# JinPLu/VeloxSeg

Hardware: AMD Instinct MI355X
Metric: training patches/s on 128^3 2-mod volumes (fwd+loss+bwd+allreduce+AdamW) (higher is better)
Workload: dtype f32

## Files before the change

include/veloxseg_hip.h:

```cpp
#ifndef VELOXSEG_HIP_H
#define VELOXSEG_HIP_H

#ifdef __cplusplus
extern "C" {
#endif

#define VX_ABI_VERSION 1

int vx_abi_version(void);
const char* vx_last_error(void);

int vx_conv3d_fwd(const float* x, const float* x2, int C1, const float* w, const float* bias, float* y,
                  int B, int Cin, int Di, int Hi, int Wi, int Cout, int K, int S, int P, int G, int ps, void* stream);
int vx_conv3d_bwd_data(const float* dy, const float* w, const float* bias_like, float* dx, float* dx2, int C1,
                       int B, int Cin, int Di, int Hi, int Wi, int Cout, int K, int S, int P, int G, int ps,
                       int accumulate, void* stream);
int vx_conv3d_bwd_weight(const float* x, const float* x2, int C1, const float* dy, float* dw, float* db,
                         int B, int Cin, int Di, int Hi, int Wi, int Cout, int K, int S, int P, int G, int ps, void* stream);

int vx_conv3d_bwd_weight_tiled(const float* x, const float* x2, int C1, const float* dy, float* dw, float* db,
                               int B, int Cin, int Di, int Hi, int Wi, int Cout, int K, int S, int P, int G, int ps, void* stream);
int vx_down_wgrad_ws_floats(int B, int Cin, int Di, int Hi, int Wi, int Cout);
int vx_down_wgrad_mfma(const float* x, const float* dy, float* dw, float* db, float* ws, long ws_floats,
                       int B, int Cin, int Di, int Hi, int Wi, int Cout, void* stream);
// ... 223 lines not shown
                       const void* seed_ptr, unsigned long long dstream, float p_drop, void* mbits, void* stream);
int vx_pwa_attn_bwd_mb(const float* q, const float* k, const float* v, const float* table, const float* out, const float* lse, const float* dout,
                       float* dq, float* dk, float* dv, float* dtable, float* delta_ws, const VxPwaPlan* plan, int B, int M, int cq, int cv,
                       const void* seed_ptr, unsigned long long dstream, float p_drop, const void* mbits, void* stream);
int vx_pwa_attn_bwd_nofold_mb(const float* q, const float* k, const float* v, const float* table, const float* out, const float* lse, const float* dout,
                              float* dq, float* dk, float* dv, float* delta_ws, const VxPwaPlan* plan, int B, int M, int cq, int cv,
                              const void* seed_ptr, unsigned long long dstream, float p_drop, const void* mbits, void* stream);
int vx_pwa_attn_mfma_ok(const VxPwaPlan* plan, int B, int M, int cq, int cv);
int vx_pwa_attn_set_mfma(int on);
int vx_pwa_attn_bwd1h_ok(const VxPwaPlan* plan, int B, int M, int cq, int cv);
int vx_pwa_attn_set_f16_bwd(int on);
int vx_pwa_attn_set_f16_bwd_ragged(int on);
int vx_pwa_attn_set_f16_bwd_m1(int on);
int vx_pwa_attn_set_short(int on);

int vx_seg_loss_fwd(const float* l0, const float* l1, const float* l2, const float* l3, int nh, const void* labels, int lab_kind,
                    double* acc, int B, int C, long V, void* stream);
int vx_sqdiff_sum(const float* a, const float* b, long n, double* acc, void* stream);
int vx_sqdiff_sum_bs(const float* a, const float* b, long n_per_sample, long b_batch_stride, int B, double* acc, void* stream);
int vx_mse_bwd_bs(const float* a, const float* b, long n_per_sample, long b_batch_stride, int B, const float* coef, const float* gout, float* da, void* stream);
int vx_sqdiff_sum_grad_bs(const float* a, const float* b, long n_per_sample, long b_batch_stride, int B, double* acc, float scale, float* da, void* stream);
int vx_sqdiff_sum_grad_bs_h(const void* a, const float* b, long n_per_sample, long b_batch_stride, int B, double* acc, float scale, void* da, int a_h16, void* stream);
int vx_loss_finalize(const double* seg_acc, int nh, int B, int C, long V, const float* head_weights,
                     const double* rc_acc, long n_rc, float w_rc,
                     const float* gram_seg, const float* g0, const float* g1, const float* g2, const float* g3, int M, int Cg, float w_f,
                     float* loss_out, float* coef, void* stream);
int vx_seg_loss_bwd(const float* logits, const void* labels, int lab_kind, const float* coef_head, const float* gout,
                    float* dlogits, int B, int C, long V, void* stream);
int vx_seg_loss_bwd4(const float* lg0, const float* lg1, const float* lg2, const float* lg3, int nh, const void* labels, int lab_kind, const float* coef,
                     int coef_stride, const float* gout, float* dl0, float* dl1, float* dl2, float* dl3, int B, int C, long V, void* stream);
int vx_seg_loss_ds_ok(int C, int D, int H, int W);
int vx_seg_loss_ds_set_columns(int on);
int vx_seg_loss_ds_ws_floats(const int* low_dims, int nh, int B, int C, int D);
int vx_seg_loss_ds_fwd(const float* l0, const float* l1, const float* l2, const float* l3, const int* low_dims, int nh, const void* labels, int lab_kind,
                       double* acc, int B, int C, int D, int H, int W, void* stream);
int vx_seg_loss_ds_bwd(const float* l0, const float* l1, const float* l2, const float* l3, const int* low_dims, int nh, const void* labels, int lab_kind,
                       const float* coef, int coef_stride, const float* gout, float* dl0, float* dl1, float* dl2, float* dl3, float* ws,
                       int B, int C, int D, int H, int W, void* stream);
int vx_seg_loss_ds_h16_ok(const int* low_dims, int nh, int B, int C, int D, int H, int W);
int vx_seg_loss_ds_fwd_h(const void* l0, const float* l1, const float* l2, const float* l3, const int* low_dims, int nh, const void* labels, int lab_kind,
                         double* acc, int B, int C, int D, int H, int W, int l0_h16, void* stream);
int vx_seg_loss_ds_bwd_h(const void* l0, const float* l1, const float* l2, const float* l3, const int* low_dims, int nh, const void* labels, int lab_kind,
                         const float* coef, int coef_stride, const float* gout, void* dl0, float* dl1, float* dl2, float* dl3, float* ws,
                         int B, int C, int D, int H, int W, int l0_h16, void* stream);
int vx_mse_bwd(const float* a, const float* b, const float* coef, const float* gout, float* da, long n, void* stream);
int vx_gram_mse_bwd(const float* gs, const float* g0, const float* g1, const float* g2, const float* g3, int M, const float* coef,
                    const float* gout, float* dgs, float* d0, float* d1, float* d2, float* d3, long n, void* stream);
int vx_gram_fwd(const float* x, float* G, int B, int C, long V, void* stream);
int vx_gram_bwd(const float* x, const float* dG, float* dx, int B, int C, long V, void* stream);
int vx_upsample_trilinear_fwd(const float* x, float* out, long BC, int d, int h, int w, int D, int H, int W, void* stream);
int vx_upsample_trilinear_bwd(const float* dout, float* dx, float* ws, long BC, int d, int h, int w, int D, int H, int W, void* stream);

int vx_upconv_set_mfma4(int on);
int vx_upconv_k2s2_fwd(const float* x, const float* w, const float* bias, float* y, int B, int Ci, int Co, int d, int h, int wd, void* stream);
int vx_upconv_k2s2_bwd_data(const float* dy, const float* w, float* dx, int B, int Ci, int Co, int d, int h, int wd, void* stream);
int vx_upconv_k2s2_wgrad_ok(int Ci, int Co);
int vx_upconv_k2s2_wgrad(const float* x, const float* dy, float* dw, int B, int Ci, int Co, int d, int h, int wd, void* stream);

int vx_adamw_step(float* p, const float* g, float* m, float* v, long n, float lr, float beta1, float beta2, float eps,
                  float weight_decay, long step, float grad_scale, void* stream);
int vx_grad_sqnorm_blocks(void);
int vx_grad_sqnorm_partials(const float* g, long n, double* ws, void* stream);
int vx_adamw_step_ex(float* p, const float* g, float* m, float* v, long n, float lr, float beta1, float beta2, float eps, float weight_decay, long step,
                     float grad_scale, const double* ws, int nws, float max_norm, float* stats, int write_stats, float* ema, float one_minus_decay,
                     const unsigned char* chunk_group, const float* group_lr, const float* group_wd, int ngroups, void* stream);

int vx_sw_extract(const float* vol, float* win, int C, int D, int H, int W, int rd, int rh, int rw, int z0, int y0, int x0, void* stream);
int vx_sw_accumulate(const float* win, float* acc, int C, int D, int H, int W, int rd, int rh, int rw, int z0, int y0, int x0, float weight, void* stream);
int vx_sw_finalize(const float* acc, float* out, unsigned char* labels, const float* cz, const float* cy, const float* cx,
                   int C, int D, int H, int W, void* stream);
#define VX_SW_MAX_WINDOWS 16
int vx_sw_extract_mirror(const float* vol, float* win, const int* table, int nwin, int mask, int B, int C, int D, int H, int W, int rd, int rh, int rw, void* stream);
int vx_sw_mirror_sum(const float* pred, float* wsum, long rows, int rd, int rh, int rw, int mask, int first, void* stream);
int vx_sw_mirror_accumulate(const float* pred, const float* wsum, float* acc, int C, int D, int H, int W, int rd, int rh, int rw, int z0, int y0, int x0,
                            int mask, float weight, void* stream);
int vx_sw_blend_accumulate(const float* pred, const float* wsum, float* acc, const float* g, float floor, int C, int D, int H, int W, int rd, int rh, int rw,
                           int z0, int y0, int x0, int mask, float weight, void* stream);
int vx_sw_blend_finalize(const float* acc, float* out, unsigned char* labels, const float* gc, float floor, const int* tab, int cz, int cy, int cx,
                         int C, int D, int H, int W, void* stream);
int vx_argmax_channels(const float* logits, unsigned char* labels, int B, int C, long V, void* stream);
int vx_confusion(const void* pred, int pred_bytes, const void* gt, int gt_bytes, unsigned long long* conf, int B, long V, int NC, void* stream);

int vx_min_value(const float* x, long n, float* out_init_inf, void* stream);
int vx_bbox_gt(const float* x, float thr, int C, int D, int H, int W, int* out6, void* stream);
int vx_label_chunk_count(const void* labels, int lab_bytes, long n, int chunk, int fg, int* counts, void* stream);
int vx_label_kth_in_chunk(const void* labels, int lab_bytes, long n, long chunk_start, int chunk, int fg, int k, long* out_index, void* stream);
int vx_rotate_z(const float* x, float* out, int C, int D, int H, int W, float cos_a, float sin_a, int mode, void* stream);

#define VX_AUG_RECORD_BYTES 192
#define VX_AUG_MAX_STEPS 8
#define VX_AUG_LABEL (-1)
#define VX_AUG_NOISE_STREAM 0x564158475541ull
int vx_augment_batch(const void* records, int n_image, int n_label, float* x_out, void* y_out, int label_bytes, int B, int M, int D, int H, int W, void* stream);

int vx_moments_blocks(void);
int vx_moments_ws_doubles(void);
int vx_moments_partials(const float* x, long n, const float* thr, const void* mask, int mask_bytes, const double* center, double* ws, void* stream);
int vx_moments_reduce(const double* ws, double* acc, int accumulate, double* stats, int phase, void* stream);
int vx_moments_stats(const float* x, long n, const float* thr, double* ws, double* stats, void* stream);
int vx_normalize_apply(const float* x, float* out, long n, const float* thr, const double* stats, float mean, float std, int clip, float lo, float hi,
                       int policy, float floor, void* stream);
int vx_key_histogram(const float* x, const void* mask, int mask_bytes, long n, long prefix, int prefix_bits, int bin_bits, unsigned long long* hist,
                     unsigned int* minmax_key, unsigned long long* nan_count, void* stream);
int vx_resample_axes(const float* x, float* out, int C, int D, int H, int W, int Do, int Ho, int Wo, const int* i0, const int* i1, const float* w, int mode, void* stream);
int vx_resample_axes_label(const void* x, void* out, int lab_bytes, int C, int D, int H, int W, int Do, int Ho, int Wo, const int* i0, void* stream);
int vx_native_argmax(const float* logits, unsigned char* labels, int C, int D, int H, int W, int Do, int Ho, int Wo, const int* i0, const int* i1, const float* w, void* stream);

int vx_cc_ws_bytes(int D, int H, int W);
int vx_cc_grid_cap(void);
int vx_cc_label(const void* labels, int lab_bytes, int* cc, int D, int H, int W, int connectivity, void* ws, int* num, void* stream);
int vx_cc_tally(const int* cc, const void* other, int other_bytes, long V, int N, unsigned long long* sizes, unsigned long long* hits, void* stream);
int vx_cc_select(const int* cc, const unsigned char* keep, int N, const void* in, void* out, int lab_bytes, long V, void* stream);

int vx_conv_mfma_ok(int Cin, int Cout, int D, int H, int W, int K, int S, int P, int G, int ps);
int vx_conv_mfma_set_stem_f16(int on);
int vx_conv_mfma_set_stem_pieces(int np);
int vx_conv_mfma_stem_pieces(void);
int vx_conv_mfma_ws_floats(int Cin, int Cout, int K, int backward);
int vx_conv_mfma_fwd(const float* x, const float* w, const float* bias, float* y, float* ws, int B, int Cin, int D, int H, int W, int Cout, int K, int S, int P,
                     void* stream);
int vx_conv_mfma_fwd_writes_absmax(int Cin, int Cout, int D, int H, int W, int K, int S, int P);
int vx_conv_mfma_fwd_mx(const float* x, const float* w, const float* bias, float* y, float* ws, unsigned* x_absmax, int B, int Cin, int D, int H, int W, int Cout,
                        int K, int S, int P, void* stream);
int vx_conv_mfma_bwd_data(const float* dy, const float* w, float* dx, float* ws, int B, int Cin, int D, int H, int W, int Cout, int K, int S, int P, int accumulate,
                          void* stream);

int vx_expand_split_ws_floats(int Cc, int ns);
int vx_expand_fwd_mfma_split(const float* x, const float* w, const float* bias, float* wt_ws, float* y, int B, int Cc, int D, int H, int W, int ns, void* stream);
int vx_expand_bwd_data_mfma_split(const float* dy_fine, const float* w, float* wt_ws, float* dx, int B, int Cc, int D, int H, int W, int accumulate, int ns, void* stream);
int vx_expand_split_ew_offset(int Cc);
int vx_expand_prep_split22(const float* w, float* wt_fwd, float* wt_bwd, int Cc, void* stream);
int vx_expand_fwd_mfma_split_prepared(const float* x, const float* bias, const float* wt_fwd, float* y, int B, int Cc, int D, int H, int W, void* stream);
int vx_expand_bwd_data_mfma_split_prepared(const float* dy_fine, const float* wt_bwd, const float* ew_fwd, float* dx, int B, int Cc, int D, int H, int W, int accumulate, void* stream);
int vx_expand_bwd_data_mfma_split_ew(const float* dy_fine, const float* w, float* wt_ws, float* dx, int B, int Cc, int D, int H, int W, int accumulate, int ns,
                                     const float* ew_fwd, void* stream);

int vx_ln_pw_ok(int C, int NS, const int* J, long V, int s2d);
int vx_ln_pw_tiles(int B, long V);
int vx_ln_pw_fwd(const void* const* ptrs, int M, int NS, const int* J, int B, int C, long V, float eps, int s2d, int gd, int gh, int gw, void* stream);
int vx_ln_pw_bwd(const void* const* ptrs, int M, int NS, const int* J, int B, int C, long V, float eps, int s2d, int gd, int gh, int gw, void* stream);
int vx_pwa_post_ok(int C, int Cv, int R, long V);
int vx_pwa_post_tiles(int B, long V);
int vx_pwa_post_fwd(const void* const* ptrs, int M, int B, int C, int Cv, int R, long V, float eps, float alpha, const void* seed_ptr, float p_mix, float p_ffn, void* stream);
int vx_pwa_post_bwd(const void* const* ptrs, int M, int B, int C, int Cv, int R, long V, float eps, float alpha, const void* seed_ptr, float p_mix, float p_ffn, void* stream);

int vx_inmlp_ok(int C, int R, long V);
int vx_inmlp_tiles(long V);
int vx_inmlp_fwd(const float* o, const double* part, int nparts, float* stats, const float* w1, const float* b1, const float* w2, const float* b2, float* out,
                 int B, int C, int R, long V, float eps, const void* seed_ptr, unsigned long long site, float p_drop, void* stream);
int vx_inmlp_bwd(const float* o, const float* stats, const float* w1, const float* b1, const float* w2, const float* dout, float* dn, float* part_dn,
                 float* sc_n, float* sc_h, float* sc_da, float* sc_dz, int B, int C, int R, long V, const void* seed_ptr, unsigned long long site, float p_drop,
                 void* stream);
int vx_pw_wgrad_group(const void* const* ptrs, const long* dims, int nj, const void* const* fptrs, const int* fdims, int nf, void* stream);

typedef struct VxTape VxTape;
int vx_tape_build(void* hip_graph, int max_lanes, VxTape** out);
int vx_tape_build_pgo(void* graph, int max_lanes, const float* dur_us, int n, VxTape** out);
int vx_tape_info(const VxTape* tape, int* n_nodes, int* n_kernels, int* n_lanes, int* n_events);
int vx_tape_set_lane_rotation(VxTape* tape, int k);
int vx_tape_replay(VxTape* tape, void* stream);
int vx_tape_free(VxTape* tape);
int vx_tape_flag_set(void* flag, int value, void* stream);
int vx_tape_flag_wait(const void* flag, int value, void* stream);
int vx_tape_set_flags(int on);
int vx_tape_set_flag_timeout_ms(int ms);
int vx_tape_flag_timeouts(void);
int vx_tape_hop(int slot, void* src, void* dst);
int vx_tape_mark(int id, void* stream);
int vx_tape_wait_marker(VxTape* tape, int id, void* stream);
int vx_tape_has_marker(const VxTape* tape, int id);
int vx_tape_profile(VxTape* tape, void* stream, int reps, float* us);
int vx_tape_describe(const VxTape* tape, int* lane, int* grid, int* waits4, char* names, int name_stride);
int vx_tape_waits(const VxTape* tape, int* waits, int stride);
int vx_tape_launch_node(VxTape* tape, int node, void* stream);
int vx_tape_set_fuzz(int seed, float max_us, float prob);
int vx_tape_node_param(const VxTape* tape, int node, int k, int nparams, int size, void* out, int cap, int* got);
int vx_tape_node_kind(const VxTape* tape, int node);
int vx_tape_replay_prefix(VxTape* tape, void* stream, int k);
int vx_tape_lane_stream(void* any_stream, int lane, void** out);
int vx_spin_us(float us, void* stream);
int vx_tape_lanes_distinct(void);
int vx_tape_spin_us(void);
int vx_tape_lane_on_caller_queue(void);
int vx_tape_permute_lanes(const int* perm4);

#ifdef __cplusplus
}
#endif
#endif
```

veloxseg_amd/csrc/pointwise.hip:

```cpp
#include "vx_common.h"
#include "../../include/veloxseg_hip.h"
#include <type_traits>

typedef float vx_f32x4 __attribute__((ext_vector_type(4)));

template <typename TX>
__device__ __forceinline__ const TX* vx_pw_row(const TX* __restrict__ x, const TX* __restrict__ x2, int C1, int Cin, int b, int c, long V) {
    return (c < C1) ? x + ((long)b * C1 + c) * V : x2 + ((long)b * (Cin - C1) + (c - C1)) * V;
}

struct VxPwEpi {
    int mode;
    float* aux;
    VxDrop drop;
    float alpha;
};
__device__ __forceinline__ float vx_pw_epi(const VxPwEpi& e, float val, long idx) {
    if (e.mode == 1) { e.aux[idx] = val; return vx_gelu(val) * vx_drop(e.drop, (uint64_t)idx); }
    if (e.mode == 2) return val * vx_drop(e.drop, (uint64_t)idx) * vx_gelu_grad(e.aux[idx]);
    if (e.mode == 3) return fmaf(e.alpha, e.aux[idx], val * vx_drop(e.drop, (uint64_t)idx));
    return val;
}
static inline VxPwEpi vx_no_epi() { VxPwEpi e; e.mode = 0; e.aux = nullptr; e.drop.seed_ptr = nullptr; e.drop.stream = 0; e.drop.p = 0.0f; e.alpha = 1.0f; return e; }

// ... 663 lines not shown
        float4 bv[4];
#pragma unroll
        for (int s = 0; s < 4; ++s) {
            const int k = k0 + 4 * s + q;
            const bool k_ok = k < kend;
            av[s] = (m_ok && k_ok) ? wrow[(long)k * wsk] : 0.0f;
            const float* srow = (k < S1) ? src + ((long)b * S1 + k) * V : src2 + ((long)b * (Kch - S1) + (k - S1)) * V;
            bv[s] = (v_ok && k_ok) ? *reinterpret_cast<const float4*>(srow + v_b) : make_float4(0.f, 0.f, 0.f, 0.f);
        }
#pragma unroll
        for (int s = 0; s < 4; ++s) {
            acc[0] = __builtin_amdgcn_mfma_f32_16x16x4f32(av[s], bv[s].x, acc[0], 0, 0, 0);
            acc[1] = __builtin_amdgcn_mfma_f32_16x16x4f32(av[s], bv[s].y, acc[1], 0, 0, 0);
            acc[2] = __builtin_amdgcn_mfma_f32_16x16x4f32(av[s], bv[s].z, acc[2], 0, 0, 0);
            acc[3] = __builtin_amdgcn_mfma_f32_16x16x4f32(av[s], bv[s].w, acc[3], 0, 0, 0);
        }
    }
    if (ksplit > 1) {
#pragma unroll
        for (int j = 0; j < 4; ++j)
#pragma unroll
            for (int reg = 0; reg < 4; ++reg) vx_ksum4[wave][(j * 4 + reg) * 64 + lane] = acc[j][reg];
        __syncthreads();
        if (wave != 0 || !live) return;
#pragma unroll
        for (int j = 0; j < 4; ++j)
#pragma unroll
            for (int reg = 0; reg < 4; ++reg) {
                const int e = (j * 4 + reg) * 64 + lane;
                acc[j][reg] = (vx_ksum4[0][e] + vx_ksum4[1][e]) + (vx_ksum4[2][e] + vx_ksum4[3][e]);
            }
    }
    if (!v_ok) return;
#pragma unroll
    for (int reg = 0; reg < 4; ++reg) {
        const int m = mt * 16 + 4 * q + reg;
        if (m < Mch) {
            float* drow = (m < D1) ? dst + ((long)b * D1 + m) * V : dst2 + ((long)b * (Mch - D1) + (m - D1)) * V;
            const float bb = bias ? bias[m] : 0.0f;
            float4 o = make_float4(acc[0][reg] + bb, acc[1][reg] + bb, acc[2][reg] + bb, acc[3][reg] + bb);
            if (epi.mode) {
                const long idx = ((long)b * Mch + m) * V + v_b;
                if (epi.mode == 1) *reinterpret_cast<float4*>(epi.aux + idx) = o;
                const float4 ax = epi.mode >= 2 ? *reinterpret_cast<const float4*>(epi.aux + idx) : o;
                if (epi.mode == 3) {
                    o.x = fmaf(epi.alpha, ax.x, o.x * vx_drop(epi.drop, (uint64_t)idx));
                    o.y = fmaf(epi.alpha, ax.y, o.y * vx_drop(epi.drop, (uint64_t)idx + 1));
                    o.z = fmaf(epi.alpha, ax.z, o.z * vx_drop(epi.drop, (uint64_t)idx + 2));
                    o.w = fmaf(epi.alpha, ax.w, o.w * vx_drop(epi.drop, (uint64_t)idx + 3));
                } else if (epi.mode == 1) {
                    o.x = vx_gelu(ax.x) * vx_drop(epi.drop, (uint64_t)idx);
                    o.y = vx_gelu(ax.y) * vx_drop(epi.drop, (uint64_t)idx + 1);
                    o.z = vx_gelu(ax.z) * vx_drop(epi.drop, (uint64_t)idx + 2);
                    o.w = vx_gelu(ax.w) * vx_drop(epi.drop, (uint64_t)idx + 3);
                } else {
                    o.x = o.x * vx_drop(epi.drop, (uint64_t)idx) * vx_gelu_grad(ax.x);
                    o.y = o.y * vx_drop(epi.drop, (uint64_t)idx + 1) * vx_gelu_grad(ax.y);
                    o.z = o.z * vx_drop(epi.drop, (uint64_t)idx + 2) * vx_gelu_grad(ax.z);
                    o.w = o.w * vx_drop(epi.drop, (uint64_t)idx + 3) * vx_gelu_grad(ax.w);
                }
            }
            float4* dp = reinterpret_cast<float4*>(drow + v_b);
            if (accumulate) { const float4 old = *dp; o.x += old.x; o.y += old.y; o.z += old.z; o.w += old.w; }
            *dp = o;
        }
    }
}
__global__ void __launch_bounds__(256) vx_pw_mfma4_k(const float* __restrict__ src, const float* __restrict__ src2, int S1,
                                                     const float* __restrict__ w, int wsm, int wsk, const float* __restrict__ bias,
                                                     float* __restrict__ dst, float* __restrict__ dst2, int D1,
                                                     int Mch, int Kch, long V, int B, int n_vt, int accumulate, int ksplit, VxPwEpi epi) {
    vx_pw_mfma4_body(blockIdx.x, blockIdx.y, src, src2, S1, w, wsm, wsk, bias, dst, dst2, D1, Mch, Kch, V, B, n_vt, accumulate, ksplit, epi);
}

static int vx_pw_mfma4_enabled = 1;
extern "C" int vx_pw_mfma_set_wide(int on) { vx_pw_mfma4_enabled = on ? 1 : 0; return 0; }

static inline int vx_pw_ksplit(long wave_tiles, int Kch) { return (wave_tiles < 2048 && Kch >= 64) ? 4 : 1; }

static int vx_pw_conv_mfma_impl(const float* src, const float* src2, int S1, const float* w, int transpose_w, const float* bias,
                                float* dst, float* dst2, int D1, int B, int Mch, int Kch, int Cin_of_w, long V, int accumulate, void* stream, const VxPwEpi& epi) {
    VX_REQUIRE(src && w && dst && B > 0 && Mch > 0 && Kch > 0 && V > 0, "vx_pw_conv_mfma: bad args");
    if (S1 <= 0 || S1 > Kch) S1 = Kch;
    if (D1 <= 0 || D1 > Mch) D1 = Mch;
    VX_REQUIRE((S1 == Kch || src2) && (D1 == Mch || dst2), "vx_pw_conv_mfma: second tensor of a concat is missing");
    const int wsm = transpose_w ? 1 : Cin_of_w, wsk = transpose_w ? Cin_of_w : 1;
    if ((V & 3) == 0 && vx_pw_mfma4_enabled) {
        const int n_vt4 = vx_cdiv(V, 64);
        const int ks4 = vx_pw_ksplit((long)B * n_vt4 * vx_cdiv(Mch, 16), Kch);
        dim3 g4(ks4 > 1 ? (unsigned)((long)B * n_vt4) : vx_cdiv((long)B * n_vt4, 4), vx_cdiv(Mch, 16));
        vx_pw_mfma4_k<<<g4, 256, 0, (hipStream_t)stream>>>(src, src2, S1, w, wsm, wsk, bias, dst, dst2, D1, Mch, Kch, V, B, n_vt4, accumulate, ks4, epi);
        VX_LAUNCH_CHECK("vx_pw_conv_mfma");
        return 0;
    }
    const int n_vt = vx_cdiv(V, 16);
    const int ksplit = vx_pw_ksplit((long)B * n_vt * vx_cdiv(Mch, 16), Kch);
    dim3 grid(ksplit > 1 ? (unsigned)((long)B * n_vt) : vx_cdiv((long)B * n_vt, 4), vx_cdiv(Mch, 16));
    vx_pw_mfma_k<<<grid, 256, 0, (hipStream_t)stream>>>(src, src2, S1, w, wsm, wsk, bias, dst, dst2, D1, Mch, Kch, V, B, n_vt, accumulate, 0, 0, 0, 0, ksplit, epi);
    VX_LAUNCH_CHECK("vx_pw_conv_mfma");
    return 0;
}

extern "C" int vx_pw_conv_mfma(const float* src, const float* src2, int S1, const float* w, int transpose_w, const float* bias,
                               float* dst, float* dst2, int D1, int B, int Mch, int Kch, int Cin_of_w, long V, int accumulate, void* stream) {
    return vx_pw_conv_mfma_impl(src, src2, S1, w, transpose_w, bias, dst, dst2, D1, B, Mch, Kch, Cin_of_w, V, accumulate, stream, vx_no_epi());
}

__global__ void __launch_bounds__(256) vx_pw_bwd_fused_k(const float* __restrict__ dy, const float* __restrict__ w, float* __restrict__ dx, float* __restrict__ dx2,
                                                         int C1, int Cin, int Cout, long V, int B, int n_vt, int accumulate, int ksplit, int n1, int gx1,
                                                         const float* __restrict__ x, const float* __restrict__ x2, float* __restrict__ dw, float* __restrict__ db,
                                                         int vox_per_wave, int chunks_per_b, int n_ci_tiles, int gx2) {
    const int id = blockIdx.x;
    if (id < n1) {
        VxPwEpi e; e.mode = 0; e.aux = nullptr; e.drop.seed_ptr = nullptr; e.drop.stream = 0; e.drop.p = 0.0f; e.alpha = 1.0f;
        vx_pw_mfma4_body(id % gx1, id / gx1, dy, nullptr, Cout, w, 1, Cin, nullptr, dx, dx2, C1, Cin, Cout, V, B, n_vt, accumulate, ksplit, e);
    } else {
        const int j = id - n1;
        vx_pw_wgrad_body(j % gx2, j / gx2, x, x2, C1, Cin, dy, Cout, V, B, dw, db, vox_per_wave, chunks_per_b, n_ci_tiles);
    }
}

extern "C" int vx_pw_conv_bwd_fused(const float* dy, const float* w, const float* x, const float* x2, int C1, float* dx, float* dx2, float* dw, float* db,
                                    int B, int Cin, int Cout, long V, int accumulate, void* stream) {
    VX_REQUIRE(dy && w && x && dx && dw && B > 0 && Cin > 0 && Cout > 0 && V > 0, "vx_pw_conv_bwd_fused: bad args");
    if (C1 <= 0 || C1 > Cin) C1 = Cin;
    VX_REQUIRE(C1 == Cin || (x2 && dx2), "vx_pw_conv_bwd_fused: second tensor of a concat is missing");
    if ((V & 3) != 0 || !vx_pw_mfma4_enabled) {
        if (int e = vx_pw_conv_mfma_impl(dy, nullptr, 0, w, 1, nullptr, dx, dx2, C1, B, Cin, Cout, Cin, V, accumulate, stream, vx_no_epi())) return e;
        return vx_pw_conv_bwd_weight(x, x2, C1, dy, dw, db, B, Cin, Cout, V, stream);
    }
    const int n_vt4 = vx_cdiv(V, 64);
    const int ks4 = vx_pw_ksplit((long)B * n_vt4 * vx_cdiv(Cin, 16), Cout);
    const int gx1 = ks4 > 1 ? (int)((long)B * n_vt4) : vx_cdiv((long)B * n_vt4, 4), gy1 = vx_cdiv(Cin, 16);
    const int mt = vx_cdiv(Cout, 16), nt = vx_cdiv(Cin, 16);
    long waves_per_tile = 1024 / ((long)mt * nt);
    if (waves_per_tile < 4) waves_per_tile = 4;
    long vpw = ((long)B * V + waves_per_tile - 1) / waves_per_tile;
    vpw = (vpw + 63) / 64 * 64;
    if (vpw < 256) vpw = 256;
    const int chunks_per_b = vx_cdiv(V, vpw);
    const int gx2 = vx_cdiv((long)B * chunks_per_b, 4), gy2 = mt * nt;
    const long n1 = (long)gx1 * gy1, n2 = (long)gx2 * gy2;
    VX_REQUIRE(n1 + n2 < 0x7fffffffL, "vx_pw_conv_bwd_fused: grid too large");
    vx_pw_bwd_fused_k<<<dim3((unsigned)(n1 + n2)), 256, 0, (hipStream_t)stream>>>(dy, w, dx, dx2, C1, Cin, Cout, V, B, n_vt4, accumulate, ks4, (int)n1, gx1,
                                                                               x, x2, dw, db, (int)vpw, chunks_per_b, nt, gx2);
    VX_LAUNCH_CHECK("vx_pw_conv_bwd_fused");
    return 0;
}

struct VxWgJob { const float* x; const float* dy; float* dw; float* db; int Cin, Cout; long V; int B, vpw, chunks_per_b, nt, gx, blk0, nblk; };
struct VxFoldJob { const float* part; float* dg; float* dbeta; int C, rows, blk0, nblk; };
#define VX_WGG_JOBS 24
#define VX_WGG_FOLDS 16
struct VxWgGroup { VxWgJob j[VX_WGG_JOBS]; VxFoldJob f[VX_WGG_FOLDS]; int nj, nf; };
__global__ void __launch_bounds__(256) vx_pw_wgrad_group_k(VxWgGroup g) {
    const int id = blockIdx.x;
    for (int k = 0; k < g.nj; ++k) {
        const VxWgJob& J = g.j[k];
        if (id >= J.blk0 && id < J.blk0 + J.nblk) {
            const int l = id - J.blk0;
            vx_pw_wgrad_body<float>(l % J.gx, l / J.gx, J.x, (const float*)nullptr, J.Cin, J.Cin, J.dy, J.Cout, J.V, J.B, J.dw, J.db, J.vpw, J.chunks_per_b, J.nt);
            return;
        }
    }
    for (int k = 0; k < g.nf; ++k) {
        const VxFoldJob& F = g.f[k];
        if (id >= F.blk0 && id < F.blk0 + F.nblk) {
            const int r0 = (id - F.blk0) * 64, r1 = min(F.rows, r0 + 64), n = 2 * F.C;
            const int P = n < 256 ? n : 256, G = 256 / P;
            const int ci = threadIdx.x % P, gi = threadIdx.x / P;
            if (gi >= G) return;
            for (int i = ci; i < n; i += P) {
                float acc = 0.0f;
                int rr = r0 + gi;
                for (; rr + 7 * G < r1; rr += 8 * G) {
                    float t[8];
#pragma unroll
                    for (int u = 0; u < 8; ++u) t[u] = F.part[(long)(rr + u * G) * n + i];
                    acc += ((t[0] + t[1]) + (t[2] + t[3])) + ((t[4] + t[5]) + (t[6] + t[7]));
                }
                for (; rr < r1; rr += G) acc += F.part[(long)rr * n + i];
                atomicAdd(i < F.C ? F.dg + i : F.dbeta + (i - F.C), acc);
            }
            return;
        }
    }
}

extern "C" int vx_pw_wgrad_group(const void* const* ptrs, const long* dims, int nj, const void* const* fptrs, const int* fdims, int nf, void* stream) {
    VX_REQUIRE(nj >= 0 && nj <= VX_WGG_JOBS && nf >= 0 && nf <= VX_WGG_FOLDS && (nj + nf) > 0 && (nj == 0 || (ptrs && dims)) && (nf == 0 || (fptrs && fdims)), "vx_pw_wgrad_group: bad args");
    VxWgGroup g = {};
    g.nj = nj; g.nf = nf;
    long blk = 0;
    for (int k = 0; k < nj; ++k) {
        VxWgJob& J = g.j[k];
        J.x = (const float*)ptrs[4 * k]; J.dy = (const float*)ptrs[4 * k + 1]; J.dw = (float*)ptrs[4 * k + 2]; J.db = (float*)ptrs[4 * k + 3];
        J.Cin = (int)dims[4 * k]; J.Cout = (int)dims[4 * k + 1]; J.V = dims[4 * k + 2]; J.B = (int)dims[4 * k + 3];
        VX_REQUIRE(J.x && J.dy && J.dw && J.Cin > 0 && J.Cout > 0 && J.V > 0 && J.B > 0, "vx_pw_wgrad_group: bad job %d", k);
        const int mt = vx_cdiv(J.Cout, 16), nt = vx_cdiv(J.Cin, 16);
        constexpr int wgg_waves = 1024, wgg_minv = 256;
        long waves_per_tile = wgg_waves / ((long)mt * nt);
        if (waves_per_tile < 4) waves_per_tile = 4;
        long vpw = ((long)J.B * J.V + waves_per_tile - 1) / waves_per_tile;
        vpw = (vpw + 63) / 64 * 64;
        if (vpw < wgg_minv) vpw = wgg_minv;
        J.vpw = (int)vpw; J.chunks_per_b = vx_cdiv(J.V, vpw); J.nt = nt;
        J.gx = vx_cdiv((long)J.B * J.chunks_per_b, 4);
        J.blk0 = (int)blk; J.nblk = J.gx * mt * nt;
        blk += J.nblk;
    }
    for (int k = 0; k < nf; ++k) {
        VxFoldJob& F = g.f[k];
        F.part = (const float*)fptrs[3 * k]; F.dg = (float*)fptrs[3 * k + 1]; F.dbeta = (float*)fptrs[3 * k + 2];
        F.C = fdims[2 * k]; F.rows = fdims[2 * k + 1];
        VX_REQUIRE(F.part && F.dg && F.dbeta && F.C > 0 && F.rows > 0, "vx_pw_wgrad_group: bad fold %d", k);
        F.blk0 = (int)blk; F.nblk = vx_cdiv(F.rows, 64);
        blk += F.nblk;
    }
    VX_REQUIRE(blk < 0x7fffffffL, "vx_pw_wgrad_group: grid too large");
    vx_pw_wgrad_group_k<<<dim3((unsigned)blk), 256, 0, (hipStream_t)stream>>>(g);
    VX_LAUNCH_CHECK("vx_pw_wgrad_group");
    return 0;
}

template <int CIT>
__global__ void __launch_bounds__(256) vx_pw_bwd_fused_big_k(const float* __restrict__ dy, const float* __restrict__ w, float* __restrict__ dx, float* __restrict__ dx2,
                                                             int C1, int Cin, int Cout, long V, int B, int accumulate, int n1, int gx1, int gy1,
                                                             const float* __restrict__ x, const float* __restrict__ x2, float* __restrict__ dw, float* __restrict__ db,
                                                             int vox_per_wave, int chunks_per_b, int n_ci_tiles, int gx2) {
    const int id = blockIdx.x;
    if (id < n1) {
        VxPwEpi e; e.mode = 0; e.aux = nullptr; e.drop.seed_ptr = nullptr; e.drop.stream = 0; e.drop.p = 0.0f; e.alpha = 1.0f;
        const int bx = id % gx1, t = id / gx1;
        vx_pw_bwd_data_body<CIT>(bx, t % gy1, t / gy1, dy, w, dx, dx2, C1, Cin, Cout, V, accumulate, e);
    } else {
        const int j = id - n1;
        vx_pw_wgrad_body(j % gx2, j / gx2, x, x2, C1, Cin, dy, Cout, V, B, dw, db, vox_per_wave, chunks_per_b, n_ci_tiles);
    }
}

extern "C" int vx_pw_conv_bwd_fused_big(const float* dy, const float* w, const float* x, const float* x2, int C1, float* dx, float* dx2, float* dw, float* db,
                                        int B, int Cin, int Cout, long V, int accumulate, void* stream) {
    VX_REQUIRE(dy && w && x && dx && dw && B > 0 && Cin > 0 && Cout > 0 && V > 0, "vx_pw_conv_bwd_fused_big: bad args");
    VX_REQUIRE(Cin % 4 == 0, "vx_pw_conv_bwd_fused_big: Cin must be a multiple of 4 (got %d)", Cin);
    if (C1 <= 0 || C1 > Cin) C1 = Cin;
    VX_REQUIRE(C1 == Cin || (x2 && dx2), "vx_pw_conv_bwd_fused_big: second tensor of a concat is missing");
    int T = (Cin % 16 == 0) ? 16 : (Cin % 8 == 0) ? 8 : 4;
    while (T > 4 && (C1 % T)) T >>= 1;
    while (T > 4 && (long)vx_cdiv(V, 256) * (Cin / T) * B < 512) T >>= 1;
    VX_REQUIRE(C1 % T == 0, "vx_pw_conv_bwd_fused_big: concat split must be a multiple of 4");
    const int gx1 = vx_cdiv(V, 256), gy1 = Cin / T;
    const long n1 = (long)gx1 * gy1 * B;
    const int mt = vx_cdiv(Cout, 16), nt = vx_cdiv(Cin, 16);
    long waves_per_tile = 1024 / ((long)mt * nt);
    if (waves_per_tile < 4) waves_per_tile = 4;
    long vpw = ((long)B * V + waves_per_tile - 1) / waves_per_tile;
    vpw = (vpw + 63) / 64 * 64;
    if (vpw < 256) vpw = 256;
    const int chunks_per_b = vx_cdiv(V, vpw);
    const int gx2 = vx_cdiv((long)B * chunks_per_b, 4);
    const long n2 = (long)gx2 * mt * nt;
    VX_REQUIRE(n1 + n2 < 0x7fffffffL, "vx_pw_conv_bwd_fused_big: grid too large");
    hipStream_t st = (hipStream_t)stream;
    const dim3 grid((unsigned)(n1 + n2));
    switch (T) {
        case 16: vx_pw_bwd_fused_big_k<16><<<grid, 256, 0, st>>>(dy, w, dx, dx2, C1, Cin, Cout, V, B, accumulate, (int)n1, gx1, gy1, x, x2, dw, db, (int)vpw, chunks_per_b, nt, gx2); break;
        case 8: vx_pw_bwd_fused_big_k<8><<<grid, 256, 0, st>>>(dy, w, dx, dx2, C1, Cin, Cout, V, B, accumulate, (int)n1, gx1, gy1, x, x2, dw, db, (int)vpw, chunks_per_b, nt, gx2); break;
        default: vx_pw_bwd_fused_big_k<4><<<grid, 256, 0, st>>>(dy, w, dx, dx2, C1, Cin, Cout, V, B, accumulate, (int)n1, gx1, gy1, x, x2, dw, db, (int)vpw, chunks_per_b, nt, gx2); break;
    }
    VX_LAUNCH_CHECK("vx_pw_conv_bwd_fused_big");
    return 0;
}

extern "C" int vx_pw_conv_gelu_fwd(const float* x, const float* w, const float* bias, float* a, float* h, int B, int Cin, int Cout, long V, int mfma,
                                   const void* seed_ptr, unsigned long long dstream, float p, void* stream) {
    VX_REQUIRE(x && w && a && h && a != h, "vx_pw_conv_gelu_fwd: bad args");
    VxPwEpi e; e.mode = 1; e.aux = a; e.drop = vx_mk_drop(seed_ptr, dstream, p); e.alpha = 1.0f;
    if (mfma) return vx_pw_conv_mfma_impl(x, nullptr, Cin, w, 0, bias, h, nullptr, 0, B, Cout, Cin, Cin, V, 0, stream, e);
    return vx_pw_conv_fwd_impl(x, nullptr, Cin, w, bias, h, B, Cin, Cout, V, stream, e);
}
extern "C" int vx_pw_conv_gelu_bwd_data(const float* dy, const float* w, const float* a, float* da, int B, int Cin, int Cout, long V, int mfma,
                                        const void* seed_ptr, unsigned long long dstream, float p, void* stream) {
    VX_REQUIRE(dy && w && a && da && a != da, "vx_pw_conv_gelu_bwd_data: bad args");
    VxPwEpi e; e.mode = 2; e.aux = const_cast<float*>(a); e.drop = vx_mk_drop(seed_ptr, dstream, p); e.alpha = 1.0f;
    if (mfma) return vx_pw_conv_mfma_impl(dy, nullptr, 0, w, 1, nullptr, da, nullptr, Cin, B, Cin, Cout, Cin, V, 0, stream, e);
    return vx_pw_conv_bwd_data_impl(dy, w, da, nullptr, Cin, B, Cin, Cout, V, 0, stream, e);
}

extern "C" int vx_pw_conv_res_fwd(const float* x, const float* w, const float* bias, const float* res, float* out, int B, int Cin, int Cout, long V, int mfma,
                                  float alpha, const void* seed_ptr, unsigned long long dstream, float p, void* stream) {
    VX_REQUIRE(x && w && res && out, "vx_pw_conv_res_fwd: bad args");
    VxPwEpi e; e.mode = 3; e.aux = const_cast<float*>(res); e.drop = vx_mk_drop(seed_ptr, dstream, p); e.alpha = alpha;
    if (mfma) return vx_pw_conv_mfma_impl(x, nullptr, Cin, w, 0, bias, out, nullptr, 0, B, Cout, Cin, Cin, V, 0, stream, e);
    return vx_pw_conv_fwd_impl(x, nullptr, Cin, w, bias, out, B, Cin, Cout, V, stream, e);
}

template <int BWD>
__global__ void __launch_bounds__(256) vx_upconv_mfma4_k(const float* __restrict__ src, const float* __restrict__ w, const float* __restrict__ bias, float* __restrict__ dst,
                                                         int Ci, int Co, int cd, int ch, int cw, int B, int n_vt, int ksplit) {
    __shared__ float vx_ksum4[4][16 * 64];
    const int Mch = BWD ? Ci : Co * 8, Kch = BWD ? Co * 8 : Ci;
    const long V = (long)cd * ch * cw;
    const int lane = threadIdx.x & 63;
    const int wave = __builtin_amdgcn_readfirstlane((int)(threadIdx.x >> 6));
    const int ks = ksplit > 1 ? wave : 0;
    const long tile_raw = ksplit > 1 ? (long)blockIdx.x : (long)blockIdx.x * 4 + wave;
    const bool live = tile_raw < (long)B * n_vt;
    if (!live && ksplit == 1) return;
    const long tile = live ? tile_raw : 0;
    const int b = (int)(tile / n_vt);
    const long v0 = (tile % n_vt) * 64;
    const int mt = blockIdx.y;
    const int r = lane & 15, q = lane >> 4;
    const int m_a = mt * 16 + r;
    const bool m_ok = m_a < Mch;
    const long v_b = v0 + 4 * r;
    const bool v_ok = v_b < V;
    const long vc = v_ok ? v_b : 0;
    const int xw = (int)(vc % cw), xh = (int)((vc / cw) % ch), xd = (int)(vc / ((long)cw * ch));
    const long fH = 2L * ch, fW = 2L * cw;
    const long fbase = ((long)(2 * xd) * fH + 2 * xh) * fW + 2 * xw;
    const int kper = ksplit > 1 ? ((Kch + 4 * 16 - 1) / (4 * 16)) * 16 : Kch;
    const int kbeg = ks * kper, kend = min(Kch, kbeg + kper);
    vx_f32x4 acc[4];
#pragma unroll
    for (int j = 0; j < 4; ++j) acc[j] = (vx_f32x4){0.f, 0.f, 0.f, 0.f};
    const float* __restrict__ wrow = w + (BWD ? (long)(m_ok ? m_a : 0) * Kch : (long)(m_ok ? m_a : 0));
    const long wsk = BWD ? 1 : (long)Co * 8;
    for (int k0 = kbeg; k0 < kend; k0 += 16) {
        float av[4];
        float4 bv[4];
#pragma unroll
        for (int s = 0; s < 4; ++s) {
            const int k = k0 + 4 * s + q;
            const bool k_ok = k < kend;
            av[s] = (m_ok && k_ok) ? wrow[(long)k * wsk] : 0.0f;
            if (BWD) {
                const int kc = k_ok ? k : 0;
                const int co = kc >> 3, tp = kc & 7;
                const float* __restrict__ fp_ = src + ((long)b * Co + co) * (8 * V) + fbase + (long)(tp >> 2) * fH * fW + (long)((tp >> 1) & 1) * fW;
                float4 lo = make_float4(0.f, 0.f, 0.f, 0.f), hi = lo;
                if (v_ok && k_ok) { lo = *reinterpret_cast<const float4*>(fp_); hi = *reinterpret_cast<const float4*>(fp_ + 4); }
                bv[s] = (tp & 1) ? make_float4(lo.y, lo.w, hi.y, hi.w) : make_float4(lo.x, lo.z, hi.x, hi.z);
            } else {
                bv[s] = (v_ok && k_ok) ? *reinterpret_cast<const float4*>(src + ((long)b * Ci + k) * V + v_b) : make_float4(0.f, 0.f, 0.f, 0.f);
            }
        }
#pragma unroll
        for (int s = 0; s < 4; ++s) {
            acc[0] = __builtin_amdgcn_mfma_f32_16x16x4f32(av[s], bv[s].x, acc[0], 0, 0, 0);
            acc[1] = __builtin_amdgcn_mfma_f32_16x16x4f32(av[s], bv[s].y, acc[1], 0, 0, 0);
            acc[2] = __builtin_amdgcn_mfma_f32_16x16x4f32(av[s], bv[s].z, acc[2], 0, 0, 0);
            acc[3] = __builtin_amdgcn_mfma_f32_16x16x4f32(av[s], bv[s].w, acc[3], 0, 0, 0);
        }
    }
    if (ksplit > 1) {
#pragma unroll
        for (int j = 0; j < 4; ++j)
#pragma unroll
            for (int reg = 0; reg < 4; ++reg) vx_ksum4[wave][(j * 4 + reg) * 64 + lane] = acc[j][reg];
        __syncthreads();
        if (wave != 0 || !live) return;
#pragma unroll
        for (int j = 0; j < 4; ++j)
#pragma unroll
            for (int reg = 0; reg < 4; ++reg) {
                const int e = (j * 4 + reg) * 64 + lane;
                acc[j][reg] = (vx_ksum4[0][e] + vx_ksum4[1][e]) + (vx_ksum4[2][e] + vx_ksum4[3][e]);
            }
    }
    if (!v_ok) return;
    if (BWD) {
#pragma unroll
// ... 163 lines not shown
```

Measured before the change: 1126.

## Add LDS-staged MFMA panel path for grouped pointwise weight-gradient jobs

Adds a panel mode to the grouped pointwise wgrad kernel. Up to three jobs that share the same input activation are merged into one panel, so x is read once and reused across their dy tiles. Each block stages x and dy chunks through double-buffered, swizzled LDS and accumulates with f32 MFMA, reducing across waves when there are few tiles. This aims to cut redundant global reads and improve matrix-core use, at the cost of dynamic LDS usage that limits occupancy, more atomics per chunk, and extra host-side grouping logic.

New measurement: 1130 (median of 6 runs). No clear change (+0.3%).

```diff
diff --git a/include/veloxseg_hip.h b/include/veloxseg_hip.h
--- a/include/veloxseg_hip.h
+++ b/include/veloxseg_hip.h
@@ -399,6 +399,8 @@
                  float* sc_n, float* sc_h, float* sc_da, float* sc_dz, int B, int C, int R, long V, const void* seed_ptr, unsigned long long site, float p_drop,
                  void* stream);
 int vx_pw_wgrad_group(const void* const* ptrs, const long* dims, int nj, const void* const* fptrs, const int* fdims, int nf, void* stream);
+int vx_pw_wgrad_group_set_panels(int on);
+int vx_pw_wgrad_group_set_chunk(int kb);
 
 typedef struct VxTape VxTape;
 int vx_tape_build(void* hip_graph, int max_lanes, VxTape** out);
diff --git a/veloxseg_amd/csrc/pointwise.hip b/veloxseg_amd/csrc/pointwise.hip
--- a/veloxseg_amd/csrc/pointwise.hip
+++ b/veloxseg_amd/csrc/pointwise.hip
@@ -839,9 +839,174 @@
 struct VxFoldJob { const float* part; float* dg; float* dbeta; int C, rows, blk0, nblk; };
 #define VX_WGG_JOBS 24
 #define VX_WGG_FOLDS 16
-struct VxWgGroup { VxWgJob j[VX_WGG_JOBS]; VxFoldJob f[VX_WGG_FOLDS]; int nj, nf; };
+struct VxWgPanel { int job[3]; int nm, ci0, cin, vpb, chunks_per_b, blk0, nblk; };
+struct VxWgGroup { VxWgJob j[VX_WGG_JOBS]; VxFoldJob f[VX_WGG_FOLDS]; VxWgPanel p[VX_WGG_JOBS]; int nj, nf, np; };
+
+#define VX_WGP_TILES 8
+#define VX_WGP_OUT 16
+typedef const __attribute__((address_space(1))) vx_f32x4* vx_gcf4;
+
+__device__ __forceinline__ void vx_lds_bar() {
+    __builtin_amdgcn_fence(__ATOMIC_RELEASE, "workgroup", "local");
+    __builtin_amdgcn_s_barrier();
+    __builtin_amdgcn_fence(__ATOMIC_ACQUIRE, "workgroup", "local");
+}
+
+__device__ __forceinline__ void vx_wgp_flush(int t, vx_f32x4 a4, float bsum, int nt, int mt0, int mt1, float* dw0, float* dw1, float* dw2, float* db0, float* db1, float* db2,
+                                             int co0, int co1, int co2, int Cin, int ci0, int cin, int q, int r) {
+    const int a = t / nt, n = t - a * nt;
+    const int m = a < mt0 ? 0 : (a < mt0 + mt1 ? 1 : 2);
+    const int mi = a - (m == 0 ? 0 : (m == 1 ? mt0 : mt0 + mt1));
+    float* const dw = m == 0 ? dw0 : (m == 1 ? dw1 : dw2);
+    float* const db = m == 0 ? db0 : (m == 1 ? db1 : db2);
+    const int Co = m == 0 ? co0 : (m == 1 ? co1 : co2);
+#pragma unroll
+    for (int reg = 0; reg < 4; ++reg) {
+        const int row = mi * 16 + 4 * q + reg, col = n * 16 + r;
+        if (row < Co && col < cin) atomicAdd(dw + (long)row * Cin + ci0 + col, a4[reg]);
+    }
+    if (db != nullptr && n == 0 && ci0 == 0 && q == 0 && mi * 16 + r < Co) atomicAdd(db + mi * 16 + r, bsum);
+}
+
+__device__ __forceinline__ void vx_pw_wgrad_panel_body(const VxWgGroup& g, const VxWgPanel& P, const int l) {
+    extern __shared__ __attribute__((aligned(16))) float vx_wgp_lds[];
+    const int tid = threadIdx.x, lane = tid & 63, wave = __builtin_amdgcn_readfirstlane(tid >> 6);
+    const int r = lane & 15, q = lane >> 4, rr = tid >> 4;
+    const VxWgJob& J0 = g.j[P.job[0]];
+    const long V = J0.V;
+    const int Cin = J0.Cin, cin = P.cin, ci0 = P.ci0, nt = (cin + 15) >> 4;
+    const int b = l / P.chunks_per_b;
+    const long v0 = (long)(l % P.chunks_per_b) * P.vpb, v1 = (v0 + P.vpb < V) ? v0 + P.vpb : V;
+    const VxWgJob& J1 = g.j[P.job[P.nm > 1 ? 1 : 0]];
+    const VxWgJob& J2 = g.j[P.job[P.nm > 2 ? 2 : 0]];
+    const float *dy0 = J0.dy, *dy1 = J1.dy, *dy2 = J2.dy;
+    float *dw0 = J0.dw, *dw1 = J1.dw, *dw2 = J2.dw, *db0 = J0.db, *db1 = J1.db, *db2 = J2.db;
+    const int co0 = J0.Cout, co1 = P.nm > 1 ? J1.Cout : 0, co2 = P.nm > 2 ? J2.Cout : 0;
+    const int mt0 = (co0 + 15) >> 4, mt1 = (co1 + 15) >> 4, mt2 = (co2 + 15) >> 4;
+    const int mtt = mt0 + mt1 + mt2, NR = nt + mtt, T = mtt * nt;
+    const char* base[VX_WGP_TILES];
+    bool rok[VX_WGP_TILES];
+#pragma unroll
+    for (int i = 0; i < VX_WGP_TILES; ++i) {
+        const int j = i - nt;
+        const float* s_; int C, tl;
+        if (i < nt) { s_ = J0.x + ((long)b * Cin + ci0) * V; C = cin; tl = i; }
+        else if (j < mt0) { s_ = dy0 + (long)b * co0 * V; C = co0; tl = j; }
+        else if (j < mt0 + mt1) { s_ = dy1 + (long)b * co1 * V; C = co1; tl = j - mt0; }
+        else { s_ = dy2 + (long)b * co2 * V; C = co2; tl = j - mt0 - mt1; }
+        rok[i] = i < NR && 16 * tl + rr < C;
+        base[i] = reinterpret_cast<const char*>(s_ + (long)16 * tl * V + v0);
+    }
+    const unsigned loff = (unsigned)((rr * V + 4 * r) * 4);
+    const int nv = (int)(v1 - v0);
+    vx_f32x4 st[VX_WGP_TILES];
+    auto request = [&](int p) {
+        const bool vok = 64 * p + 4 * r < nv;
+#pragma unroll
+        for (int i = 0; i < VX_WGP_TILES; ++i)
+            st[i] = (rok[i] && vok) ? *(vx_gcf4)(unsigned long long)(base[i] + (loff + (unsigned)(256 * p))) : (vx_f32x4){0.f, 0.f, 0.f, 0.f};
+    };
+    auto stage = [&](float* buf) {
+#pragma unroll
+        for (int i = 0; i < VX_WGP_TILES; ++i)
+            if (i < NR) *reinterpret_cast<vx_f32x4*>(buf + (i * 16 + rr) * 64 + 4 * (r ^ rr)) = st[i];
+    };
+    const bool vsplit = T <= 4;
+    const int s_lo = vsplit ? wave : 0, s_hi = vsplit ? wave + 1 : 4;
+    int tile[4], aoff[4], boff[4];
+    bool live[4];
+    vx_f32x4 acc[4];
+    float bs[4];
+#pragma unroll
+    for (int u = 0; u < 4; ++u) {
+        tile[u] = vsplit ? u : wave + 4 * u;
+        live[u] = tile[u] < T;
+        const int a = live[u] ? tile[u] / nt : 0, n = live[u] ? tile[u] - a * nt : 0;
+        aoff[u] = ((nt + a) * 16 + r) * 64;
+        boff[u] = (n * 16 + r) * 64;
+        acc[u] = (vx_f32x4){0.f, 0.f, 0.f, 0.f};
+        bs[u] = 0.0f;
+    }
+    auto compute = [&](const float* buf) {
+        for (int s = s_lo; s < s_hi; ++s) {
+            const int slot = 4 * ((4 * s + q) ^ r);
+#pragma unroll
+            for (int u = 0; u < 4; ++u) {
+                if (live[u]) {
+                    const vx_f32x4 av = *reinterpret_cast<const vx_f32x4*>(buf + aoff[u] + slot);
+                    const vx_f32x4 bv = *reinterpret_cast<const vx_f32x4*>(buf + boff[u] + slot);
+                    bs[u] += (av[0] + av[1]) + (av[2] + av[3]);
+                    acc[u] = __builtin_amdgcn_mfma_f32_16x16x4f32(av[0], bv[0], acc[u], 0, 0, 0);
+                    acc[u] = __builtin_amdgcn_mfma_f32_16x16x4f32(av[1], bv[1], acc[u], 0, 0, 0);
+                    acc[u] = __builtin_amdgcn_mfma_f32_16x16x4f32(av[2], bv[2], acc[u], 0, 0, 0);
+                    acc[u] = __builtin_amdgcn_mfma_f32_16x16x4f32(av[3], bv[3], acc[u], 0, 0, 0);
+                }
+            }
+        }
+    };
+    float* const buf0 = vx_wgp_lds;
+    float* const buf1 = vx_wgp_lds + NR * 1024;
+    const int np = (nv + 63) >> 6;
+    request(0);
+    stage(buf0);
+    vx_lds_bar();
+    int p = 0;
+    for (; p + 1 < np; ++p) {
+        request(p + 1);
+        compute((p & 1) ? buf1 : buf0);
+        stage((p & 1) ? buf0 : buf1);
+        vx_lds_bar();
+    }
+    compute((p & 1) ? buf1 : buf0);
+    auto flush = [=](int t, vx_f32x4 a4, float bsum) {
+        vx_wgp_flush(t, a4, bsum, nt, mt0, mt1, dw0, dw1, dw2, db0, db1, db2, co0, co1, co2, Cin, ci0, cin, q, r);
+    };
+#pragma unroll
+    for (int u = 0; u < 4; ++u) {
+        bs[u] += __shfl_xor(bs[u], 16, 64);
+        bs[u] += __shfl_xor(bs[u], 32, 64);
+    }
+    if (!vsplit) {
+#pragma unroll
+        for (int u = 0; u < 4; ++u)
+            if (live[u]) flush(tile[u], acc[u], bs[u]);
+        return;
+    }
+    float* const red = vx_wgp_lds;
+    float* const bsr = vx_wgp_lds + 16 * 256;
+    vx_lds_bar();
+#pragma unroll
+    for (int u = 0; u < 4; ++u) {
+        if (live[u]) {
+#pragma unroll
+            for (int reg = 0; reg < 4; ++reg) red[(wave * 4 + u) * 256 + reg * 64 + lane] = acc[u][reg];
+            if (q == 0) bsr[(wave * 4 + u) * 16 + r] = bs[u];
+        }
+    }
+    vx_lds_bar();
+    if (wave < T) {
+        vx_f32x4 s4;
+#pragma unroll
+        for (int reg = 0; reg < 4; ++reg)
+            s4[reg] = (red[(0 * 4 + wave) * 256 + reg * 64 + lane] + red[(1 * 4 + wave) * 256 + reg * 64 + lane]) +
+                      (red[(2 * 4 + wave) * 256 + reg * 64 + lane] + red[(3 * 4 + wave) * 256 + reg * 64 + lane]);
+        const float bsum = (bsr[(0 * 4 + wave) * 16 + r] + bsr[(1 * 4 + wave) * 16 + r]) + (bsr[(2 * 4 + wave) * 16 + r] + bsr[(3 * 4 + wave) * 16 + r]);
+        flush(wave, s4, bsum);
+    }
+}
+
+template <bool PANELS>
 __global__ void __launch_bounds__(256) vx_pw_wgrad_group_k(VxWgGroup g) {
     const int id = blockIdx.x;
+    if constexpr (PANELS) {
+        for (int k = 0; k < g.np; ++k) {
+            const VxWgPanel& P = g.p[k];
+            if (id >= P.blk0 && id < P.blk0 + P.nblk) {
+                vx_pw_wgrad_panel_body(g, P, id - P.blk0);
+                return;
+            }
+        }
+    }
     for (int k = 0; k < g.nj; ++k) {
         const VxWgJob& J = g.j[k];
         if (id >= J.blk0 && id < J.blk0 + J.nblk) {
@@ -874,16 +1039,64 @@
     }
 }
 
+static int vx_wgg_panels = 1, vx_wgg_chunk_kb = 0;
+#define VX_WGP_MIN_BV 8192
+extern "C" int vx_pw_wgrad_group_set_panels(int on) { vx_wgg_panels = on < 0 ? 0 : (on > 2 ? 2 : on); return 0; }
+extern "C" int vx_pw_wgrad_group_set_chunk(int kb) { vx_wgg_chunk_kb = kb > 0 ? kb : 0; return 0; }
+
 extern "C" int vx_pw_wgrad_group(const void* const* ptrs, const long* dims, int nj, const void* const* fptrs, const int* fdims, int nf, void* stream) {
     VX_REQUIRE(nj >= 0 && nj <= VX_WGG_JOBS && nf >= 0 && nf <= VX_WGG_FOLDS && (nj + nf) > 0 && (nj == 0 || (ptrs && dims)) && (nf == 0 || (fptrs && fdims)), "vx_pw_wgrad_group: bad args");
     VxWgGroup g = {};
-    g.nj = nj; g.nf = nf;
+    g.nj = nj; g.nf = nf; g.np = 0;
     long blk = 0;
+    size_t lds = 0;
     for (int k = 0; k < nj; ++k) {
         VxWgJob& J = g.j[k];
         J.x = (const float*)ptrs[4 * k]; J.dy = (const float*)ptrs[4 * k + 1]; J.dw = (float*)ptrs[4 * k + 2]; J.db = (float*)ptrs[4 * k + 3];
         J.Cin = (int)dims[4 * k]; J.Cout = (int)dims[4 * k + 1]; J.V = dims[4 * k + 2]; J.B = (int)dims[4 * k + 3];
         VX_REQUIRE(J.x && J.dy && J.dw && J.Cin > 0 && J.Cout > 0 && J.V > 0 && J.B > 0, "vx_pw_wgrad_group: bad job %d", k);
+    }
+    bool taken[VX_WGG_JOBS] = {};
+    auto eligible = [&](int k) {
+        const VxWgJob& J = g.j[k];
+        return vx_wgg_panels && (J.V & 3) == 0 && J.V <= (1L << 24) && (((uintptr_t)J.x | (uintptr_t)J.dy) & 15) == 0 && (vx_wgg_panels == 2 || (long)J.B * J.V >= VX_WGP_MIN_BV);
+    };
+    for (int k = 0; k < nj; ++k) {
+        if (taken[k] || !eligible(k)) continue;
+        const VxWgJob& J = g.j[k];
+        const int nt = vx_cdiv(J.Cin, 16);
+        int mt = vx_cdiv(J.Cout, 16), mem[3] = {k, 0, 0}, nm = 1, nsplit = 1;
+        for (int k2 = k + 1; k2 < nj && nm < 3; ++k2) {
+            const VxWgJob& J2 = g.j[k2];
+            if (taken[k2] || !eligible(k2) || J2.x != J.x || J2.Cin != J.Cin || J2.V != J.V || J2.B != J.B) continue;
+            const int mt2 = vx_cdiv(J2.Cout, 16);
+            if (nt + mt + mt2 > VX_WGP_TILES || (mt + mt2) * nt > VX_WGP_OUT) continue;
+            mem[nm++] = k2; mt += mt2;
+        }
+        while (nsplit <= 8 && (vx_cdiv(nt, nsplit) + mt > VX_WGP_TILES || vx_cdiv(nt, nsplit) * mt > VX_WGP_OUT)) nsplit *= 2;
+        if (nsplit > 8 || g.np + nsplit > VX_WGG_JOBS) continue;
+        const int nts = vx_cdiv(nt, nsplit), rows = 16 * (nts + mt);
+        const long kb = vx_wgg_chunk_kb > 0 ? vx_wgg_chunk_kb : 128;
+        long vpb = (kb * 256 / rows + 63) / 64 * 64;
+        if (vpb < 64) vpb = 64;
+        if (vpb > (1L << 24)) vpb = 1L << 24;
+        for (int s = 0; s < nsplit && 16 * nts * s < J.Cin; ++s) {
+            VxWgPanel& P = g.p[g.np++];
+            for (int m = 0; m < 3; ++m) P.job[m] = mem[m];
+            P.nm = nm; P.ci0 = 16 * nts * s; P.cin = (J.Cin - P.ci0 < 16 * nts) ? J.Cin - P.ci0 : 16 * nts;
+            P.vpb = (int)vpb; P.chunks_per_b = vx_cdiv(J.V, vpb);
+            P.blk0 = (int)blk; P.nblk = J.B * P.chunks_per_b;
+            blk += P.nblk;
+            const int T = vx_cdiv(P.cin, 16) * mt;
+            size_t need = (size_t)(vx_cdiv(P.cin, 16) + mt) * 8192;
+            if (T <= 4 && need < (size_t)(16 * 256 + 16 * 16) * 4) need = (size_t)(16 * 256 + 16 * 16) * 4;
+            if (need > lds) lds = need;
+        }
+        for (int m = 0; m < nm; ++m) taken[mem[m]] = true;
+    }
+    for (int k = 0; k < nj; ++k) {
+        VxWgJob& J = g.j[k];
+        if (taken[k]) { J.blk0 = 0; J.nblk = 0; continue; }
         const int mt = vx_cdiv(J.Cout, 16), nt = vx_cdiv(J.Cin, 16);
         constexpr int wgg_waves = 1024, wgg_minv = 256;
         long waves_per_tile = wgg_waves / ((long)mt * nt);
@@ -905,7 +1118,16 @@
         blk += F.nblk;
     }
     VX_REQUIRE(blk < 0x7fffffffL, "vx_pw_wgrad_group: grid too large");
-    vx_pw_wgrad_group_k<<<dim3((unsigned)blk), 256, 0, (hipStream_t)stream>>>(g);
+    if (g.np == 0) {
+        vx_pw_wgrad_group_k<false><<<dim3((unsigned)blk), 256, 0, (hipStream_t)stream>>>(g);
+    } else {
+        static bool attr = false;
+        if (!attr) {
+            VX_REQUIRE(hipFuncSetAttribute((const void*)vx_pw_wgrad_group_k<true>, hipFuncAttributeMaxDynamicSharedMemorySize, VX_WGP_TILES * 8192) == hipSuccess, "vx_pw_wgrad_group: LDS attribute");
+            attr = true;
+        }
+        vx_pw_wgrad_group_k<true><<<dim3((unsigned)blk), 256, lds, (hipStream_t)stream>>>(g);
+    }
     VX_LAUNCH_CHECK("vx_pw_wgrad_group");
     return 0;
 }
```
